# ygtxr1997/MSML

Measured on AMD Instinct MI355X. Metric: images/sec (112x112) ires50-MSML+PartialFC training step, higher is better.
Workload: dtype bf16; 1 GPU; iresnet50-MSML (OSB r18 + FM x4) + 85742-id ArcFace PartialFC, 112x112, batch 256/GPU, fwd+bwd+clip+SGD; global_batch=256, parallelism=dp1+class-parallel head, launch=eager, weight gradients + OSB on side streams

## Files before the change

include/msml_hip.h:

```cpp
#ifndef MSML_HIP_H
#define MSML_HIP_H

#include <stddef.h>
#include <stdint.h>

#ifdef __cplusplus
extern "C" {
#endif

#define MSML_ABI_VERSION 1

enum { MSML_F32 = 0, MSML_BF16 = 1, MSML_BF16X3 = 2 };

enum {
  MSML_OK = 0,
  MSML_ERR_SHAPE = -1,
  MSML_ERR_DTYPE = -2,
  MSML_ERR_LAUNCH = -3,
  MSML_ERR_UNSUPPORTED = -4,
  MSML_ERR_WORKSPACE = -5
};

enum { MSML_ACT_TANH = 0, MSML_ACT_SIGMOID = 1 };
enum { MSML_ARITH_ADD = 0, MSML_ARITH_SUB = 1, MSML_ARITH_MUL = 2, MSML_ARITH_DIV = 3 };
// ... 88 lines not shown
                          int accumulate, long M, int C, const void* next_x, const float* next_mean,
                          const float* next_invstd, double* next_acc, int dtype, void* stream);
int msml_bn_act_bwd_acc(const void* dy, const void* x, const float* scale, const float* shift,
                        const float* alpha, const float* save_mean, const float* save_invstd,
                        const void* residual_first, const void* add, void* dx, void* dres, float* dgamma,
                        float* dbeta, float* dalpha, int accumulate, long M, int C, double* acc, int dtype,
                        void* stream);
int msml_bn_act_bwd(const void* dy, const void* x, const float* scale, const float* shift,
                    const float* alpha, const float* save_mean, const float* save_invstd,
                    const void* residual_first, void* dx, void* dres, float* dgamma, float* dbeta,
                    float* dalpha, int accumulate, long M, int C, float* workspace, long ws_floats,
                    int dtype, void* stream);
int msml_bias_grad(const void* dy, long M, int Cp, int Creal, float* db, int accumulate,
                   float* workspace, long ws_floats, int dtype, void* stream);
int msml_add(const void* a, const void* b, void* out, long n, int dtype, void* stream);

int msml_dap_fwd(const void* x, float* seg, unsigned char* mask, int N, int H, int W, int Cp,
                 int dtype, void* stream);
int msml_dap_bwd(const float* dseg, void* dx, int N, int H, int W, int Cp, int dtype, void* stream);
int msml_seg_consensus_loss(const float* logit, const long* msk, int N, int H, int W, float alpha,
                            float beta, float* loss, float* dlogit, float* workspace,
                            long ws_floats, void* stream);
int msml_seg_consensus_loss_r(const float* logit, const long* msk, int N, int H, int W, float alpha, float beta,
                              int reduce_pixel_all, int reduce_pixel_kl_all, float* loss, float* dlogit,
                              float* workspace, long ws_floats, void* stream);

int msml_rownorm_fwd(const float* w, int R, int Rp, int E, void* dst, int ld, float* inv_norm,
                     int dtype, void* stream);
int msml_rownorm_bwd(const float* w, const float* inv_norm, const float* dy, int ldy, int R, int E,
                     float* dw, int accumulate, void* stream);
int msml_gather_target(const float* cosm, int ld, const long* label, int N, float* out,
                       void* stream);
int msml_margin_fwd(float* cosm, const long* label, int N, int C, int ld, int kind, float s,
                    float m, float a, float k, void* stream);
int msml_margin_bwd(const float* dlogit, int ldg, const long* label, const float* cos_t, int N,
                    int C, void* dcos, int ldo, int kind, float s, float m, float a, float k,
                    int dtype, void* stream);
int msml_pfc_rowstats(const float* cosm, int ld, int N, int C, const long* label, int kind, float s,
                      float m, float a, float k, float* rowmax, float* rowsum, void* stream);
int msml_pfc_grad(const float* cosm, int ld, int N, int C, const long* label, int kind, float s,
                  float m, float a, float k, const float* gmax, const float* gsum, float eps_ls,
                  float inv_n, void* dcos, int ldo, float* ptarget, int dtype, void* stream);
int msml_sgd_momentum(float* w, const float* grad, float* mom, long n, float lr, float mu, float wd,
                      int first_step, const float* clip_coef, void* stream);
int msml_grad_norm_clip(const float* grad, long n, float max_norm, float* out2, float* workspace,
                        long ws_floats, void* stream);
int msml_sgd_momentum_dev(float* w, const float* grad, float* mom, long n, const float* lr, float mu, float wd,
                          const float* coef, void* stream);
int msml_grad_norm_clip_scaled(const float* grad, long n, float max_norm, float scale, float* out2, float* workspace,
                               long ws_floats, void* stream);

long msml_gemm_splitk_workspace(int M, int coutp, int K);
int msml_gemm_splitk(const void* a, int M, int K, const void* wp, int kop, float* out, int coutp,
                     void* workspace, long ws_bytes, int dtype, void* stream);

int msml_pack_weights_batched(const long* table, int count, int dtype, void* stream);
int msml_pack_tiles(int A, int B, int R, int S);
int msml_pack_weights_tiled(const long* table, const int* tile_prefix, int count, int total_tiles,
                            int dtype, void* stream);

int msml_transpose(const void* src, int R, int C, int ld_s, void* dst, int ld_d, int dtype,
                   void* stream);

int msml_conv2d_fused(const void* in0, int c0p, const void* in1, int c1p, const void* wp, int kop,
                      const float* scale, const float* shift, const float* alpha,
                      const void* residual, int res_first, void* out, int coutp, int N, int H,
                      int W, int P, int Q, int R, int S, int stride, int pad_h, int pad_w,
                      int transposed, void* stream);

int msml_conv2d_x3(const void* in0, int c0p, const void* in1, int c1p, const void* wp, int kop,
                   const float* scale, const float* shift, const float* alpha, const void* residual,
                   int res_first, void* out, int coutp, int N, int H, int W, int P, int Q, int R, int S,
                   int stride, int pad_h, int pad_w, int transposed, void* stream);
int msml_conv2d_x3_border(const void* in0, int c0p, const void* wp, int kop, const float* scale,
                          const float* shift9, const float* alpha, const void* residual, int res_first,
                          void* out, int coutp, int N, int H, int W, void* stream);
int msml_x3_bn_act_fwd(const void* x, const float* scale, const float* shift, const float* alpha,
                       const void* residual, int res_first, void* y, long M, int C, void* stream);
int msml_x3_fm_fuse_fwd(const void* x, const void* yf, void* z, long M, int C, int act, int arith,
                        void* stream);
int msml_x3_add(const void* a, const void* b, void* out, long M, int C, void* stream);
int msml_x3_from_f32(const float* src, void* dst, long M, int C, void* stream);
int msml_x3_to_f32(const void* src, float* dst, long M, int C, void* stream);

int msml_pair_sqdist(const float* emb, int n_pairs, int E, double* dist, void* stream);
int msml_pair_sqdist_f64(const double* emb, int n_pairs, int E, double* dist, void* stream);
int msml_pair_hist(const double* dist, const unsigned char* same, int n_pairs, const double* thr, int nthr,
                   int nfolds, int* hist, void* stream);

int msml_occ_draw(long seed, long offset, int N, int H, int W, int mode, int lo, int hi, int flip, int* desc,
                  void* stream);
int msml_occ_apply(const unsigned char* src, const int* desc, float* img, long* msk, float* ori, int N, int H,
                   int W, int light, void* stream);

int msml_occ_draw_tex(long seed, long offset, int N, int H, int W, int mode, int lo, int hi, int flip,
                      const int* meta, int nsets, int* desc, void* stream);
int msml_occ_resize(const unsigned char* atlas, const int* meta, const int* dir, const int* rtab, const int* desc,
                    unsigned char* patch, long patch_stride, int N, int lds_bytes, void* stream);
int msml_occ_apply_tex(const unsigned char* src, const int* desc, const unsigned char* patch, long patch_stride,
                       float* img, long* msk, float* ori, int N, int H, int W, int light, void* stream);

int msml_deconv4_bwd_data(const void* dy, const void* wp0, const void* wp1, void* dx0, void* dx1, int N, int H,
                          void* stream);

int msml_conv2d_bnbwd_rows(int coutp, int N, int P, int Q);
int msml_conv2d_bnbwd(const void* in0, int c0p, const void* wp, int kop, void* out, int coutp,
                      int N, int H, int W, int P, int Q, int R, int S, int stride, int pad_h,
                      int pad_w, int transposed, const void* bn_x, const float* bn_scale,
                      const float* bn_shift, const float* bn_alpha, const float* bn_mean,
                      const float* bn_invstd, float* partial, int rows_cap, int* rows_used,
                      void* stream);
int msml_bn_act_bwd_apply(const void* dy, const void* x, const float* scale, const float* shift,
                          const float* alpha, const float* save_mean, const float* save_invstd,
                          const float* partial, int rows, const void* add, void* dx,
                          float* dgamma, float* dbeta, float* dalpha, int accumulate, long M,
                          int C, float* coef_ws, int dtype, void* stream);

int msml_bn_act_bwd_apply_s2(const void* dy, const void* x, const float* scale, const float* shift,
                             const float* alpha, const float* save_mean, const float* save_invstd,
                             const float* partial, int rows, const void* add, int H, int W, void* dx,
                             float* dgamma, float* dbeta, float* dalpha, int accumulate, long M,
                             int C, float* coef_ws, int dtype, void* stream);
int msml_bn_act_bwd_apply_next_s2(const void* dy, const void* x, const float* scale,
                                  const float* shift, const float* alpha, const float* save_mean,
                                  const float* save_invstd, const float* partial, int rows,
                                  const void* add, int H, int W, void* dx, float* dgamma, float* dbeta,
                                  float* dalpha, int accumulate, long M, int C, float* coef_ws,
                                  const void* next_x, const float* next_mean,
                                  const float* next_invstd, float* next_partial, int dtype,
                                  void* stream);

int msml_conv2d_bnin_applies(int c0p, int coutp, int N, int H, int W, int P, int Q, int R, int S,
                             int stride, int pad_h, int pad_w, int want_stats);
int msml_conv2d_bnin(const void* in0, int c0p, const float* in_scale, const float* in_shift,
                     const float* in_alpha, const void* wp, int kop, void* out, int coutp,
                     float* stats, int N, int H, int W, int P, int Q, int R, int S, int stride,
                     int pad_h, int pad_w, void* stream);
int msml_conv_wgrad_bnin_applies(int up, int vp, int A, int Breal, int N, int H, int W, int P, int Q,
                                 int R, int S, int stride, int pad_h, int pad_w);
int msml_conv_wgrad_bnin(const void* u, int up, const void* v, int vp, const float* x_scale,
                         const float* x_shift, const float* x_alpha, float* dw, int A, int Breal,
                         int Btot, int boff, int N, int H, int W, int P, int Q, int R, int S,
                         int stride, int pad_h, int pad_w, int accumulate, void* workspace,
                         long ws_bytes, void* stream);

#define MSML_KERNEL_MFM 2
const char* msml_conv2d_kernel(int c0p, int c1p, int coutp, int N, int H, int W, int P, int Q,
                               int R, int S, int stride, int pad_h, int pad_w, int transposed,
                               int in_dtype, int out_dtype, int want_stats);

int msml_stem_im2col(const float* x, void* out, int N, int C, int H, int W, int P, int Q, int R,
                     int S, int stride, int pad, int KP, int dtype, void* stream);

int msml_bn_act_bwd_apply_rows(long M, int C);
int msml_bn_act_bwd_apply_next(const void* dy, const void* x, const float* scale, const float* shift,
                               const float* alpha, const float* save_mean, const float* save_invstd,
                               const float* partial, int rows, const void* add, void* dx,
                               float* dgamma, float* dbeta, float* dalpha, int accumulate, long M,
                               int C, float* coef_ws, const void* next_x, const float* next_mean,
                               const float* next_invstd, float* next_partial, int dtype, void* stream);

int msml_conv2d_bnin_acc_applies(int c0p, int coutp, int N, int H, int W, int P, int Q, int R, int S, int stride,
                                 int pad_h, int pad_w);
int msml_conv2d_bnin_acc(const void* in0, int c0p, const double* acc_in, double count, const float* gamma,
                         const float* beta, float* running_mean, float* running_var, float momentum, float eps,
                         float* coef_out, const float* in_alpha, void* act_out, const void* wp, int kop, void* out,
                         int coutp, double* acc_out, int N, int H, int W, int P, int Q, int R, int S, int stride,
                         int pad_h, int pad_w, void* stream);

int msml_iblock_fwd_tables(int* nptr, int* nint, int* nflt);
int msml_iblock_fwd(const void* const* ptrs, const int* ints, const float* flts, void* stream);

int msml_probe_mfma(const void* seed, float* out, int wgs, int iters, void* stream);
int msml_probe_mfma_lds(const void* seed, float* out, int wgs, int iters, void* stream);


int msml_conv2d_mfm(const void* in0, int c0p, const void* wp, int kop, const float* bias, void* out, int coutp,
                    const void* residual, unsigned char* sel, int N, int H, int W, int P, int Q, int R, int S,
                    int stride, int pad_h, int pad_w, int dtype, void* stream);

int msml_mfm_bwd(const void* dy, const unsigned char* sel, void* dz, long M, int cp, int C, int czp, int dtype,
                 void* stream);

int msml_pool2_fwd(const void* x, void* y, int N, int H, int W, int cp, int dtype, void* stream);

int msml_pool2_bwd(const void* dy, const void* x, void* dx, int N, int H, int W, int cp, int dtype, void* stream);

int msml_template_pool(const float* feats, long n_rows, long ld, int E, int flip, const float* faceness,
                       const int* order, const int* media_start, const int* tmpl_media_start, const int* launch,
                       int n_templates, double* out, void* stream);
int msml_template_pair_score(const double* tn, int n_templates, int E, const int* r1, const int* r2, long n_pairs,
                             double* score, void* stream);
int msml_roc_blocks(int n);
int msml_roc_block_counts(const double* sorted, const unsigned char* label, int n, int* blk, void* stream);
int msml_roc_points(const double* sorted, const unsigned char* label, int n, const int* off, int* tps, int* fps,
                    void* stream);
int msml_roc_reduce_blocks(int n_points);
int msml_roc_reduce(const int* tps, const int* fps, int n_points, const double* target, int n_targets,
                    unsigned char* keep, unsigned long long* part, void* stream);
int msml_pair_cosdist(const float* emb, int n_pairs, int E, double* dist, void* stream);
int msml_pair_cosdist_f64(const double* emb, int n_pairs, int E, double* dist, void* stream);
int msml_rank_count(const double* sorted, int n, const double* q, int m, int strict, int* out, void* stream);

#ifdef __cplusplus
}
#endif
#endif
```

msml_amd/functional.py:

```python
import os
import torch

from . import _lib, ops
from ._lib import BF16, DTYPE_OF, F32, TORCH_DTYPE, call
from .ops import cpad


class _ToNHWC(torch.autograd.Function):

    @staticmethod
    def forward(ctx, x, dtype):
        return ops.to_nhwc(x.float(), dtype)

    @staticmethod
    def backward(ctx, g):
        return None, None


def to_nhwc(x, dtype):
    return _ToNHWC.apply(x, dtype)


def _slice_w(w, deconv, off, n):
    if deconv:
# ... 589 lines not shown
        e = weight.shape[0]
        dtype = DTYPE_OF[x.dtype]
        wp = ops.PACKS.get(weight, False, 0, e, 0, c, c, 0, dtype, owner=grad_param)
        xf = x.reshape(n, h * w * c)
        if dtype == BF16:
            y = ops.gemm_splitk(xf, wp, cpad(e))
        else:
            y, _ = ops.conv2d(x, None, wp, None, cpad(e), h, w, 1, 0, 0, False, out_dtype=F32)
            y = y.reshape(n, cpad(e))
        y = y[:, :e] + bias.detach()
        ctx.save_for_backward(x, weight, bias)
        ctx.grad_param = grad_param
        ctx.wp = wp
        return y.contiguous().reshape(n, 1, 1, e)

    @staticmethod
    def backward(ctx, dy):
        x, weight, bias = ctx.saved_tensors
        n, h, w, c = x.shape
        e = weight.shape[0]
        dtype = DTYPE_OF[x.dtype]
        dy = dy.contiguous().to(x.dtype)
        k = h * w * c
        dx = None
        if ctx.needs_input_grad[0]:
            if dtype == BF16:
                wpt = torch.empty(k, ops.kpad(e), dtype=x.dtype, device=x.device)
                call("msml_transpose", ctx.wp, e, k, k, wpt, ops.kpad(e), dtype)
                dxf, _ = ops.conv2d(dy, None, wpt, None, k, 1, 1, 1, 0, 0, False, real=(e, k))
                dx = dxf.reshape(n, h, w, c)
            else:
                wt = ops.PACKS.get(weight, True, 0, e, 0, c, e, 0, dtype, owner=ctx.grad_param)
                dx, _ = ops.conv2d(dy, None, wt, None, c, h, w, 1, 0, 0, True, p=h, q=w, real=(e, c))
        gp = ctx.grad_param
        inplace = ops.inplace(gp)
        dw = gp.grad.view(weight.shape) if inplace else torch.empty_like(weight)
        ops.conv_wgrad(dy, x, dw, e, c, c, 0, h, w, 1, 0, 0, accumulate=inplace)
        binplace = ops.inplace(bias)
        rows = ops.bn_stats_rows(n, e)
        wsb = ops.workspace(rows * 2 * e * 4, dy.device)
        db = bias.grad if binplace else torch.empty(e, dtype=torch.float32, device=dy.device)
        call("msml_bias_grad", dy, n, e, e, db, int(binplace), wsb, wsb.numel() // 4, dtype)
        if binplace:
            ops.grad_ready(bias)
            db = None
        if inplace:
            ops.grad_ready(gp)
            dw = None
        return dx, dw, db, None


def flat_fc(x, weight4d, bias, grad_param):
    return _FlatFc.apply(x, weight4d, bias, grad_param)


def _eval_bn_coef(bn_m, c):
    stamp = (bn_m.weight._version, bn_m.bias._version, bn_m.running_mean._version,
             bn_m.running_var._version, ops.WEIGHT_EPOCH, bn_m.weight.data_ptr())
    hit = getattr(bn_m, "_msml_eval_coef", None)
    if hit is None or hit[0] != stamp:
        coef = torch.empty(2, c, dtype=torch.float32, device=bn_m.weight.device)
        call("msml_bn_finalize", None, 0, c, 0.0, bn_m.weight, bn_m.bias, bn_m.running_mean,
             bn_m.running_var, 0.1, bn_m.eps, coef[0], coef[1], None, None)
        hit = (stamp, coef)
        bn_m._msml_eval_coef = hit
    return hit[1]


def conv_bn_eval(x0, x1, conv_m, bn_m, prelu, residual, c1, res_first):
    n, h, w, c0p = x0.shape
    cin, cout = conv_m.in_channels, conv_m.out_channels
    c0 = cin - c1
    r, s = conv_m.kernel_size
    stride, (ph, pw) = conv_m.stride[0], conv_m.padding
    coutp = cpad(cout)
    assert coutp == cout == bn_m.num_features
    wp = ops.PACKS.get(conv_m.weight, False, 0, cout, 0, cin, c0, c1, BF16)
    coef = _eval_bn_coef(bn_m, coutp)
    p = ops.conv_out_size(h, r, stride, ph, False)
    q = ops.conv_out_size(w, s, stride, pw, False)
    c1p = 0 if x1 is None else x1.shape[3]
    out = torch.empty(n, p, q, coutp, dtype=torch.bfloat16, device=x0.device)
    name = "conv_fused"
    if ops.PROFILE.on:
        name = ops.conv_label("N+bn", c0p, c1p, coutp, n, h, w, p, q, r, s, stride, ph, pw, 0, BF16, BF16, False)
    with ops.PROFILE.rec(name, 2.0 * n * p * q * cin * cout * r * s):
        call("msml_conv2d_fused", x0, c0p, x1, c1p, wp, wp.shape[0], coef[0], coef[1],
             prelu.weight if prelu is not None else None, residual, int(res_first), out, coutp,
             n, h, w, p, q, r, s, stride, ph, pw, 0)
    return out


class RawImage:

    def __init__(self, x, x3=False):
        self.raw = x
        self.dtype = torch.bfloat16
        self.x3 = x3
        self._nhwc = None

    def nhwc(self):
        if self._nhwc is None:
            self._nhwc = to_nhwc(self.raw, BF16)
        return self._nhwc

    def record_stream(self, stream):
        self.raw.record_stream(stream)


def _stem_pack(conv_m):
    w = conv_m.weight
    stamp = (w._version, ops.WEIGHT_EPOCH, w.data_ptr())
    hit = getattr(conv_m, "_msml_stem_pack", None)
    if hit is None or hit[0] != stamp:
        cout, cin, r, s = w.shape
        w2 = w.detach().permute(0, 2, 3, 1).reshape(cout, r * s * cin, 1, 1).contiguous()
        hit = (stamp, ops.pack_weight(w2, False, r * s * cin, 0, BF16))
        conv_m._msml_stem_pack = hit
    return hit[1]


class _StemConv(torch.autograd.Function):

    @staticmethod
    def forward(ctx, weight, conv_m, raw):
        cout, cin, r, s = weight.shape
        col = ops.stem_im2col(raw, r, s, conv_m.stride[0], conv_m.padding[0])
        wp = _stem_pack(conv_m)
        y, stats = ops.conv2d(col, None, wp, None, cpad(cout), 1, 1, 1, 0, 0, False, want_stats=True,
                              real=(r * s * cin, cout))
        ctx.set_materialize_grads(False)
        ctx.wparam = weight
        ctx.save_for_backward(col)
        ctx.mark_non_differentiable(stats)
        return y, stats

    @staticmethod
    def backward(ctx, dy, _dstats):
        if dy is None:
            return None, None, None
        (col,) = ctx.saved_tensors
        w = ctx.wparam
        cout, cin, r, s = w.shape
        k = r * s * cin
        dw2 = torch.empty(cout, k, 1, 1, dtype=torch.float32, device=dy.device)
        ops.conv_wgrad(dy.contiguous(), col, dw2, cout, k, k, 0, 1, 1, 1, 0, 0)
        dw = dw2.view(cout, r, s, cin).permute(0, 3, 1, 2)
        if ops.inplace(w):
            w.grad.view(w.shape).add_(dw)
            ops.grad_ready(w)
            return None, None, None
        return dw.contiguous(), None, None


def stem_conv_bn(raw, conv_m, bn_m, prelu):
    if raw.x3:
        return stem_conv_bn_x3(raw, conv_m, bn_m, prelu)
    if not bn_m.training and not torch.is_grad_enabled():
        cout, cin, r, s = conv_m.weight.shape
        col = ops.stem_im2col(raw.raw, r, s, conv_m.stride[0], conv_m.padding[0])
        wp = _stem_pack(conv_m)
        coef = _eval_bn_coef(bn_m, cpad(cout))
        n, p, q, kp = col.shape
        out = torch.empty(n, p, q, cpad(cout), dtype=torch.bfloat16, device=col.device)
        name = "conv_fused"
        if ops.PROFILE.on:
            name = ops.conv_label("N+bn", kp, 0, cpad(cout), n, p, q, p, q, 1, 1, 1, 0, 0, 0, BF16, BF16, False)
        with ops.PROFILE.rec(name, 2.0 * n * p * q * r * s * cin * cout):
            call("msml_conv2d_fused", col, kp, None, 0, wp, wp.shape[0], coef[0], coef[1],
                 prelu.weight if prelu is not None else None, None, 0, out, cpad(cout), n, p, q, p, q, 1, 1,
                 1, 0, 0, 0)
        return out
    y, stats = _StemConv.apply(conv_m.weight, conv_m, raw.raw)
    return bn_act(y, stats if stats.numel() else None, bn_m, prelu, emit_stats=True)


class SplitT:
    __slots__ = ("t", "c")
    dtype = "bf16x3"

    def __init__(self, t, c):
        self.t, self.c = t, c

    @property
    def shape(self):
        n, h, w, _ = self.t.shape
        return (n, h, w, self.c)

    @property
    def device(self):
        return self.t.device

    def detach(self):
        return self

    def record_stream(self, stream):
        self.t.record_stream(stream)

    def numel(self):
        n, h, w, _ = self.t.shape
        return n * h * w * self.c


def _x3_empty(n, h, w, cp, dev):
    return SplitT(torch.empty(n, h, w, 3 * cp, dtype=torch.bfloat16, device=dev), cp)


def x3_from_f32(x):
    n, h, w, cp = x.shape
    out = _x3_empty(n, h, w, cp, x.device)
    call("msml_x3_from_f32", x.contiguous(), out.t, n * h * w, cp)
    return out


def x3_to_f32(s):
    n, h, w, cp = s.shape
    out = torch.empty(n, h, w, cp, dtype=torch.float32, device=s.device)
    call("msml_x3_to_f32", s.t, out, n * h * w, cp)
    return out


def to_nchw_any(t, c):
    if isinstance(t, SplitT):
        t = x3_to_f32(t)
    return ops.to_nchw(t, c)


def _x3_expand(w, axis, segs):
    parts = []
    off = 0
    for c, cp_ in segs:
        ws = w.narrow(axis, off, c)
        if cp_ != c:
            pad = list(ws.shape)
            pad[axis] = cp_ - c
            ws = torch.cat((ws, ws.new_zeros(pad)), axis)
        wh = ws.to(torch.bfloat16).float()
        parts += [wh, wh, ws - wh]
        off += c
    return torch.cat(parts, axis).contiguous()


def _x3_pack(owner, key, w, transpose, segs):
    stamp = (w._version, ops.WEIGHT_EPOCH, w.data_ptr(), key)
    cache = owner.__dict__.setdefault("_msml_x3_pack", {})
    hit = cache.get(key)
    if hit is None or hit[0] != stamp:
        wexp = _x3_expand(w.detach().float(), 0 if transpose else 1, segs)
        c1 = 3 * segs[0][1]
        c2 = 3 * segs[1][1] if len(segs) > 1 else 0
        hit = (stamp, ops.pack_weight(wexp, transpose, c1, c2, BF16, stored=True))
        cache[key] = hit
    return hit[1]


def conv_x3(x0, x1, conv_m, scale, shift, alpha, residual, res_first, c1=0, weight=None, pack_key="fwd"):
    import torch.nn as nn
    deconv = isinstance(conv_m, nn.ConvTranspose2d)
    w = conv_m.weight if weight is None else weight
    cin, cout = conv_m.in_channels, conv_m.out_channels
    c0 = cin - c1
    r, s = conv_m.kernel_size
    stride, (ph, pw) = conv_m.stride[0], conv_m.padding
    n, h, wd, c0p = x0.shape
    segs = [(c0, c0p)] + ([(c1, x1.shape[3])] if x1 is not None else [])
    wp = _x3_pack(conv_m, pack_key, w, deconv, segs)
    coutp = cpad(cout)
    p = ops.conv_out_size(h, r, stride, ph, deconv)
    q = ops.conv_out_size(wd, s, stride, pw, deconv)
    out = _x3_empty(n, p, q, coutp, x0.device)
    pix = n * h * wd if deconv else n * p * q
    name = "conv_x3"
    if ops.PROFILE.on and os.environ.get("MSML_PROFILE_X3_SHAPES"):
        name = "conv_x3 c%d+%d->%d %dx%d k%dx%d s%d%s n%d" % (c0p, x1.shape[3] if x1 is not None else 0, coutp, h, wd, r, s,
                                                             stride, "T" if deconv else "", n)
    with ops.PROFILE.rec(name, 2.0 * pix * cin * cout * r * s):
        call("msml_conv2d_x3", x0.t, c0p, x1.t if x1 is not None else None, x1.shape[3] if x1 is not None else 0,
             wp, wp.shape[0], scale, shift, alpha, residual.t if residual is not None else None, int(res_first),
             out.t, coutp, n, h, wd, p, q, r, s, stride, ph, pw, int(deconv))
    return out


def _pad_vec(v, cp):
    if v.numel() == cp:
        return v.detach()
    out = torch.zeros(cp, dtype=torch.float32, device=v.device)
    out[:v.numel()] = v.detach()
    return out


def conv_bn_eval_x3(x0, x1, conv_m, bn_m, prelu, residual, c1, res_first):
    coutp = cpad(conv_m.out_channels)
    coef = _eval_bn_coef(bn_m, coutp)
    return conv_x3(x0, x1, conv_m, coef[0], coef[1], prelu.weight if prelu is not None else None, residual,
                   res_first, c1)


X3_FOLD_BN1 = os.environ.get("MSML_X3_NO_BN1_FOLD") is None
X3_FOLD_MAX_RATIO = 8.0


def _bn_stamp(bn_m):
    return (bn_m.weight._version, bn_m.bias._version, bn_m.running_mean._version, bn_m.running_var._version,
            bn_m.weight.data_ptr())


def bn_conv_bn_eval_x3(x, bn_in, conv_m, bn_m, prelu):
    n, h, w, cp = x.shape
    cout, cin = conv_m.out_channels, conv_m.in_channels
    if (not X3_FOLD_BN1 or conv_m.kernel_size != (3, 3) or conv_m.stride != (1, 1) or conv_m.padding != (1, 1)
            or conv_m.bias is not None or h < 2 or w < 2):
        return None
    coutp = cpad(cout)
    cw = conv_m.weight
    stamp = (_bn_stamp(bn_in), _bn_stamp(bn_m), cw._version, cw.data_ptr(), ops.WEIGHT_EPOCH, cp)
    hit = conv_m.__dict__.get("_msml_x3_fold")
    if hit is None or hit[0] != stamp:
        ratio = float((bn_in.running_mean.detach().abs() / (bn_in.running_var.detach() + bn_in.eps).sqrt()).max())
        if not ratio <= X3_FOLD_MAX_RATIO:
            conv_m.__dict__["_msml_x3_fold"] = (stamp, None, None)
            return None
        c_in = _eval_bn_coef(bn_in, cp).double()
        c_out = _eval_bn_coef(bn_m, coutp).double()
        wd = cw.detach().double()
# ... 370 lines not shown
```

Measured before the change: 8791 images/sec.

## Fuse stem conv with BN/PReLU via recompute-from-image kernels for fwd and bwd

Adds a dedicated stem kernel family that computes the 3x3x3->64 conv from the raw fp32 image with MFMA and uses it in four passes: a stats pass, a BN+PReLU apply pass, a backward-sums pass, and a backward pass that also does the weight gradient. The conv output is never stored; it is recomputed in each pass, so the im2col buffer and the conv-output tensor round trips to memory go away. The cost is running the tiny conv up to four times and adding a partial-sum reduce kernel for dW. The path is on by default and is limited to stem shapes with W <= 128.

```diff
diff --git a/include/msml_hip.h b/include/msml_hip.h
--- a/include/msml_hip.h
+++ b/include/msml_hip.h
@@ -264,6 +264,21 @@
 int msml_stem_im2col(const float* x, void* out, int N, int C, int H, int W, int P, int Q, int R,
                      int S, int stride, int pad, int KP, int dtype, void* stream);
 
+int msml_stem_part_rows(int N, int P, int Q);
+int msml_stem_stats(const float* img, const void* wp, int ktot, int N, int H, int W, int P, int Q, int stride,
+                    double* acc, void* stream);
+int msml_stem_bn_act_fwd(const float* img, const void* wp, int ktot, int N, int H, int W, int P, int Q,
+                         int stride, const double* acc, const float* gamma, const float* beta,
+                         float* running_mean, float* running_var, float momentum, float eps, float* coef,
+                         const float* alpha, void* x, double* acc_out, void* stream);
+int msml_stem_bn_bwd_sums(const float* img, const void* wp, int ktot, int N, int H, int W, int P, int Q,
+                          int stride, const void* dx, const float* coef, const float* alpha, double* acc,
+                          void* stream);
+int msml_stem_bn_bwd_wgrad(const float* img, const void* wp, int ktot, int N, int H, int W, int P, int Q,
+                           int stride, const void* dx, const float* coef, const float* alpha,
+                           const double* acc, float* dgamma, float* dbeta, float* dalpha, int accumulate,
+                           float* part, int part_rows, float* dw, int dw_accumulate, void* stream);
+
 int msml_bn_act_bwd_apply_rows(long M, int C);
 int msml_bn_act_bwd_apply_next(const void* dy, const void* x, const float* scale, const float* shift,
                                const float* alpha, const float* save_mean, const float* save_invstd,
diff --git a/msml_amd/csrc/stem.hip b/msml_amd/csrc/stem.hip
--- /dev/null
+++ b/msml_amd/csrc/stem.hip
@@ -0,0 +1,486 @@
+#include "common.h"
+
+enum { ST_STATS = 1, ST_FWD = 2, ST_BSUMS = 3, ST_BWG = 4 };
+
+struct StemArgs {
+  const float* img;
+  const unsigned short* wp;
+  int ktot;
+  int N, H, W, P, Q, stride;
+  int M;
+  int nblk;
+  double* stats;
+  BnIn bn;
+  unsigned short* x;
+  double* xacc;
+  const unsigned short* gout;
+  BnBwdFuse bnb;
+  float* dgamma;
+  float* dbeta;
+  float* dalpha;
+  int accumulate;
+  float* part;
+};
+
+#define STEM_TAB 0
+#define STEM_RED 2048
+#define STEM_SCR0 (2048 + 3072)
+#define STEM_XOUT 4096
+#define STEM_SCR (4096 + 2048)
+#define STEM_LDS (STEM_SCR0 + 4 * STEM_SCR)
+
+template <int MODE>
+__global__ void __launch_bounds__(256, 2) k_stem(const StemArgs p) {
+#if defined(__HIP_DEVICE_COMPILE__)
+  extern __shared__ __attribute__((aligned(16))) char smem[];
+  float* tab = reinterpret_cast<float*>(smem + STEM_TAB);
+  float* red = reinterpret_cast<float*>(smem + STEM_RED);
+  const int t = threadIdx.x, lane = t & 63, wave = t >> 6;
+  const int r32 = lane & 31, h = lane >> 5;
+  char* xout = smem + STEM_SCR0 + wave * STEM_SCR;
+  char* xin = xout + STEM_XOUT;
+  MSML_LDS_REGION(tab, 3 * 64 * 4);
+  MSML_LDS_REGION(red, 4 * 3 * 64 * 4);
+  MSML_LDS_REGION(xout, STEM_SCR);
+  auto key = [](int row) -> int { return (row >> 2) & 3; };
+
+  if (MODE == ST_FWD) {
+    bn_in_fill_acc(p.bn, tab, 64, t, 256, blockIdx.x == 0);
+    __syncthreads();
+  }
+  if (MODE == ST_BWG) {
+    const double* acc = reinterpret_cast<const double*>(p.bnb.partial);
+    if (t < 64) {
+      double s0 = 0.0, s1 = 0.0, s2 = 0.0;
+#pragma unroll
+      for (int r = 0; r < MSML_ACC_ROWS; r++) {
+        s0 += acc[(r * 3 + 0) * 64 + t];
+        s1 += acc[(r * 3 + 1) * 64 + t];
+        s2 += acc[(r * 3 + 2) * 64 + t];
+      }
+      tab[t] = (float)(s0 / (double)p.M);
+      tab[64 + t] = (float)(s1 / (double)p.M);
+      if (blockIdx.x == 0) {
+        if (p.dbeta) p.dbeta[t] = (p.accumulate ? p.dbeta[t] : 0.f) + (float)s0;
+        if (p.dgamma) p.dgamma[t] = (p.accumulate ? p.dgamma[t] : 0.f) + (float)s1;
+        if (p.dalpha) p.dalpha[t] = (p.accumulate ? p.dalpha[t] : 0.f) + (float)s2;
+      }
+    }
+    __syncthreads();
+  }
+
+  u32x4 wa[2][2];
+#pragma unroll
+  for (int i = 0; i < 2; i++)
+#pragma unroll
+    for (int kk = 0; kk < 2; kk++)
+      wa[i][kk] = *reinterpret_cast<const u32x4*>(p.wp + (long)(32 * i + r32) * p.ktot + (kk * 2 + h) * 8);
+
+  const int HW = p.H * p.W, PQ = p.P * p.Q;
+  const float rcpPQ = 1.0f / (float)PQ, rcpQ = 1.0f / (float)p.Q;
+
+  const int opl = lane >> 3;
+  const int cl = (lane & 7) ^ opl;
+  const bool has_alpha = MODE == ST_FWD ? p.bn.alpha != nullptr : p.bnb.alpha != nullptr;
+  float fsc[8], fsh[8], fal[8];
+  float k1[8], k2[8], bmu[8];
+  BnbCoef bk;
+  if (MODE == ST_FWD) {
+#pragma unroll
+    for (int j = 0; j < 8; j++) {
+      fsc[j] = tab[cl * 8 + j];
+      fsh[j] = tab[64 + cl * 8 + j];
+      fal[j] = tab[128 + cl * 8 + j];
+    }
+  }
+  if (MODE == ST_BSUMS || MODE == ST_BWG) bk = bnb_load_coef(p.bnb, cl * 8);
+  if (MODE == ST_BWG) {
+#pragma unroll
+    for (int j = 0; j < 8; j++) {
+      k1[j] = tab[cl * 8 + j];
+      k2[j] = tab[64 + cl * 8 + j];
+      bmu[j] = p.bnb.mean[cl * 8 + j];
+    }
+  }
+
+  f32x4 s1[MODE == ST_STATS ? 8 : 1], s2[MODE == ST_STATS ? 8 : 1];
+#pragma unroll
+  for (int g = 0; g < (MODE == ST_STATS ? 8 : 1); g++) s1[g] = s2[g] = f32x4{0.f, 0.f, 0.f, 0.f};
+  float bq[3][8];
+#pragma unroll
+  for (int q = 0; q < 3; q++)
+#pragma unroll
+    for (int j = 0; j < 8; j++) bq[q][j] = 0.f;
+  f32x16 dw[2];
+#pragma unroll
+  for (int i = 0; i < 2; i++)
+#pragma unroll
+    for (int e = 0; e < 16; e++) dw[i][e] = 0.f;
+
+  const int gw = blockIdx.x * 4 + wave, tw = gridDim.x * 4;
+  const int nunits = (p.nblk + 1) / 2;
+  for (int u = gw; u < nunits; u += tw) {
+#pragma unroll 1
+    for (int b = 0; b < 2; b++) {
+      const int pb = (u * 2 + b) * 32;
+      if (pb >= p.M) break;
+      u32x4 e2[(MODE == ST_BSUMS || MODE == ST_BWG) ? 4 : 1];
+      if (MODE == ST_BSUMS || MODE == ST_BWG) {
+#pragma unroll
+        for (int j = 0; j < 4; j++) {
+          const int m = pb + j * 8 + opl;
+          e2[j] = m < p.M ? *reinterpret_cast<const u32x4*>(p.gout + (long)m * 64 + cl * 8) : u32x4{0, 0, 0, 0};
+        }
+      }
+      const int m = pb + r32;
+      const bool valid = m < p.M;
+      const int mm = valid ? m : 0;
+      int n = (int)((float)mm * rcpPQ), rem = mm - n * PQ;
+      if (rem < 0) { n--; rem += PQ; } else if (rem >= PQ) { n++; rem -= PQ; }
+      int oy = (int)((float)rem * rcpQ), ox = rem - oy * p.Q;
+      if (ox < 0) { oy--; ox += p.Q; } else if (ox >= p.Q) { oy++; ox -= p.Q; }
+      const int iy0 = oy * p.stride - 1, ix0 = ox * p.stride - 1;
+      unsigned int colm = 0, okmask = 0;
+#pragma unroll
+      for (int s = 0; s < 3; s++) colm |= ((unsigned)(ix0 + s) < (unsigned)p.W ? 1u : 0u) << s;
+#pragma unroll
+      for (int r = 0; r < 3; r++) okmask |= ((unsigned)(iy0 + r) < (unsigned)p.H ? colm : 0u) << (3 * r);
+      if (!valid) okmask = 0;
+      const int base = n * 3 * HW + iy0 * p.W + ix0;
+      u32x4 xb[2];
+#pragma unroll
+      for (int kk = 0; kk < 2; kk++) {
+        float f[8];
+#pragma unroll
+        for (int e = 0; e < 8; e++) {
+          const int ka = kk * 16 + e, kb = kk * 16 + 8 + e;
+          const int ta = ka / 3, tb = kb / 3;
+          const int offa = (ka - ta * 3) * HW + (ta / 3) * p.W + (ta % 3);
+          const int offb = tb < 9 ? (kb - tb * 3) * HW + (tb / 3) * p.W + (tb % 3) : 0;
+          const int tap = h ? (tb < 9 ? tb : 31) : ta;
+          const bool ok = (okmask >> tap) & 1u;
+          const int idx = ok ? base + (h ? offb : offa) : 0;
+          const float v = p.img[idx];
+          f[e] = ok ? v : 0.f;
+        }
+#pragma unroll
+        for (int e = 0; e < 4; e++) xb[kk][e] = (unsigned int)f2bf(f[2 * e]) | ((unsigned int)f2bf(f[2 * e + 1]) << 16);
+      }
+      f32x16 acc[2];
+#pragma unroll
+      for (int i = 0; i < 2; i++)
+#pragma unroll
+        for (int e = 0; e < 16; e++) acc[i][e] = 0.f;
+#pragma unroll
+      for (int kk = 0; kk < 2; kk++)
+#pragma unroll
+        for (int i = 0; i < 2; i++)
+          acc[i] = __builtin_amdgcn_mfma_f32_32x32x16_bf16(__builtin_bit_cast(bf16x8, wa[i][kk]),
+                                                           __builtin_bit_cast(bf16x8, xb[kk]), acc[i], 0, 0, 0);
+      if (MODE == ST_STATS) {
+#pragma unroll
+        for (int i = 0; i < 2; i++)
+#pragma unroll
+          for (int g = 0; g < 4; g++)
+#pragma unroll
+            for (int j = 0; j < 4; j++) {
+              const float v = acc[i][g * 4 + j];
+              if (valid) {
+                s1[4 * i + g][j] += v;
+                s2[4 * i + g][j] += v * v;
+              }
+            }
+        continue;
+      }
+#pragma unroll
+      for (int i = 0; i < 2; i++) {
+        u32x2 pk[4];
+#pragma unroll
+        for (int g = 0; g < 4; g++) {
+          pk[g][0] = (unsigned int)f2bf(acc[i][g * 4 + 0]) | ((unsigned int)f2bf(acc[i][g * 4 + 1]) << 16);
+          pk[g][1] = (unsigned int)f2bf(acc[i][g * 4 + 2]) | ((unsigned int)f2bf(acc[i][g * 4 + 3]) << 16);
+        }
+        u32x4 ch[2];
+#pragma unroll
+        for (int e = 0; e < 2; e++) {
+          auto r01 = __builtin_amdgcn_permlane32_swap(pk[0][e], pk[1][e], false, false);
+          auto r23 = __builtin_amdgcn_permlane32_swap(pk[2][e], pk[3][e], false, false);
+          ch[0][e] = r01[0]; ch[0][2 + e] = r01[1];
+          ch[1][e] = r23[0]; ch[1][2 + e] = r23[1];
+        }
+#pragma unroll
+        for (int c = 0; c < 2; c++)
+          *reinterpret_cast<u32x4*>(xout + r32 * 128 + (((4 * i + 2 * c + h) ^ (r32 & 7)) << 4)) = ch[c];
+      }
+      if (MODE == ST_BWG) {
+#pragma unroll
+        for (int kk = 0; kk < 2; kk++)
+          *reinterpret_cast<u32x4*>(xin + r32 * 64 + (((kk * 2 + h) ^ key(r32)) << 4)) = xb[kk];
+      }
+      __builtin_amdgcn_wave_barrier();
+#pragma unroll
+      for (int j = 0; j < 4; j++) {
+        const int mo = pb + j * 8 + opl;
+        u32x4 v = *reinterpret_cast<const u32x4*>(xout + (j * 64 + lane) * 16);
+        const Vec8 y = load8<unsigned short>(reinterpret_cast<const unsigned short*>(&v));
+        if (MODE == ST_FWD) {
+          if (mo < p.M) {
+            Vec8 o;
+#pragma unroll
+            for (int q = 0; q < 8; q++) {
+              float z = y.v[q] * fsc[q] + fsh[q];
+              if (has_alpha) z = z > 0.f ? z : z * fal[q];
+              o.v[q] = z;
+            }
+            store8<unsigned short>(p.x + (long)mo * 64 + cl * 8, o);
+            const Vec8 vr = round8<unsigned short>(o);
+#pragma unroll
+            for (int q = 0; q < 8; q++) {
+              bq[0][q] += vr.v[q];
+              bq[1][q] += vr.v[q] * vr.v[q];
+            }
+          }
+        }
+        if (MODE == ST_BSUMS) {
+          if (mo < p.M) bnb_accum(bk, has_alpha, load8<unsigned short>(reinterpret_cast<const unsigned short*>(&e2[j])), y, bq);
+        }
+        if (MODE == ST_BWG) {
+          const Vec8 g = load8<unsigned short>(reinterpret_cast<const unsigned short*>(&e2[j]));
+          Vec8 o;
+#pragma unroll
+          for (int q = 0; q < 8; q++) {
+            float gg = g.v[q];
+            if (has_alpha) {
+              const float z = y.v[q] * bk.sc[q] + bk.sh[q];
+              if (z <= 0.f) gg *= bk.al[q];
+            }
+            const float xh = (y.v[q] - bmu[q]) * bk.is[q];
+            o.v[q] = mo < p.M ? bk.sc[q] * (gg - k1[q] - xh * k2[q]) : 0.f;
+          }
+          u32x4 w;
+          store8<unsigned short>(reinterpret_cast<unsigned short*>(&w), o);
+          *reinterpret_cast<u32x4*>(xout + (j * 64 + lane) * 16) = w;
+        }
+      }
+      if (MODE == ST_BWG) {
+        __builtin_amdgcn_wave_barrier();
+#pragma unroll
+        for (int st = 0; st < 2; st++) {
+          u32x4 bf, af[2];
+#pragma unroll
+          for (int e = 0; e < 8; e += 2) {
+            unsigned int lo[3], hi[3];
+#pragma unroll
+            for (int d = 0; d < 2; d++) {
+              const int px = st * 16 + h * 8 + e + d;
+              const unsigned int vb = *reinterpret_cast<const unsigned short*>(xin + px * 64 + (((r32 >> 3) ^ key(px)) << 4) + (r32 & 7) * 2);
+              unsigned int va[2];
+#pragma unroll
+              for (int i = 0; i < 2; i++) {
+                const int c = 32 * i + r32;
+                va[i] = *reinterpret_cast<const unsigned short*>(xout + px * 128 + (((c >> 3) ^ (px & 7)) << 4) + (c & 7) * 2);
+              }
+              if (d == 0) { lo[0] = vb; lo[1] = va[0]; lo[2] = va[1]; } else { hi[0] = vb; hi[1] = va[0]; hi[2] = va[1]; }
+            }
+            bf[e >> 1] = lo[0] | (hi[0] << 16);
+            af[0][e >> 1] = lo[1] | (hi[1] << 16);
+            af[1][e >> 1] = lo[2] | (hi[2] << 16);
+          }
+#pragma unroll
+          for (int i = 0; i < 2; i++)
+            dw[i] = __builtin_amdgcn_mfma_f32_32x32x16_bf16(__builtin_bit_cast(bf16x8, af[i]), __builtin_bit_cast(bf16x8, bf),
+                                                            dw[i], 0, 0, 0);
+        }
+      }
+      __builtin_amdgcn_wave_barrier();
+    }
+  }
+
+  if (MODE == ST_STATS) {
+#pragma unroll
+    for (int g = 0; g < 8; g++)
+#pragma unroll
+      for (int j = 0; j < 4; j++) {
+        const float a = wave_half_sum(s1[g][j]), b2 = wave_half_sum(s2[g][j]);
+        if (r32 == 0) {
+          red[(wave * 2 + 0) * 64 + 8 * g + 4 * h + j] = a;
+          red[(wave * 2 + 1) * 64 + 8 * g + 4 * h + j] = b2;
+        }
+      }
+    __syncthreads();
+    for (int e = t; e < 2 * 64; e += 256) {
+      const int q = e / 64, c = e % 64;
+      float sum = 0.f;
+#pragma unroll
+      for (int w = 0; w < 4; w++) sum += red[(w * 2 + q) * 64 + c];
+      stats_emit(reinterpret_cast<float*>(p.stats), 1, blockIdx.x, q, 64, c, sum);
+    }
+  }
+  if ((MODE == ST_FWD && p.xacc) || MODE == ST_BSUMS) {
+    constexpr int NQ = MODE == ST_FWD ? 2 : 3;
+#pragma unroll
+    for (int q = 0; q < NQ; q++)
+#pragma unroll
+      for (int j = 0; j < 8; j++) {
+        float a = bq[q][j];
+        a += __shfl_xor(a, 9, 64);
+        a += __shfl_xor(a, 18, 64);
+        a += __shfl_xor(a, 36, 64);
+        if (lane < 8) red[(wave * NQ + q) * 64 + 8 * cl + j] = a;
+      }
+    __syncthreads();
+    for (int e = t; e < NQ * 64; e += 256) {
+      const int q = e / 64, c = e % 64;
+      float sum = 0.f;
+#pragma unroll
+      for (int w = 0; w < 4; w++) sum += red[(w * NQ + q) * 64 + c];
+      if (MODE == ST_FWD) stats_emit(reinterpret_cast<float*>(p.xacc), 1, blockIdx.x, q, 64, c, sum);
+      else bnb_emit(p.bnb.partial, 1, blockIdx.x, q, 64, c, sum);
+    }
+  }
+  if (MODE == ST_BWG) {
+    float* tile = reinterpret_cast<float*>(smem + STEM_SCR0);
+    __syncthreads();
+    for (int w = 0; w < 4; w++) {
+      if (wave == w) {
+#pragma unroll
+        for (int i = 0; i < 2; i++)
+#pragma unroll
+          for (int g = 0; g < 4; g++)
+#pragma unroll
+            for (int j = 0; j < 4; j++) {
+              const int idx = (32 * i + 8 * g + 4 * h + j) * 32 + r32;
+              tile[idx] = (w ? tile[idx] : 0.f) + dw[i][g * 4 + j];
+            }
+      }
+      __syncthreads();
+    }
+    float* dst = p.part + (long)blockIdx.x * 2048;
+    for (int e = t; e < 2048; e += 256) dst[e] = tile[e];
+  }
+#endif
+}
+
+__global__ void __launch_bounds__(1024) k_stem_wgrad_reduce(const float* __restrict__ part, int rows, float* __restrict__ dw,
+                                                            int accumulate) {
+  __shared__ float red[32][33];
+  const int co = blockIdx.x, k = threadIdx.x & 31, sl = threadIdx.x >> 5;
+  float s = 0.f;
+  for (int r = sl; r < rows; r += 32) s += part[(long)r * 2048 + co * 32 + k];
+  red[sl][k] = s;
+  __syncthreads();
+  if (sl == 0 && k < 27) {
+    float sum = 0.f;
+#pragma unroll
+    for (int i = 0; i < 32; i++) sum += red[i][k];
+    const int tap = k / 3, c = k - tap * 3;
+    float* d = dw + co * 27 + c * 9 + tap;
+    *d = (accumulate ? *d : 0.f) + sum;
+  }
+}
+
+static int stem_cus() {
+  static int cus = 0;
+  if (!cus) {
+    int dev = 0, n = 256;
+    if (hipGetDevice(&dev) == hipSuccess) (void)hipDeviceGetAttribute(&n, hipDeviceAttributeMultiprocessorCount, dev);
+    cus = n > 0 ? n : 256;
+  }
+  return cus;
+}
+
+static int stem_grid(long M) {
+  const long nblk = (M + 31) / 32, nunits = (nblk + 1) / 2;
+  long grid = (long)stem_cus() * 4;
+  const long need = (nunits + 3) / 4;
+  if (grid > need) grid = need;
+  return (int)(grid < 1 ? 1 : grid);
+}
+
+static int stem_fill(StemArgs& a, const char* who, const float* img, const void* wp, int ktot, int N, int H, int W, int P,
+                     int Q, int stride) {
+  MSML_CHECK(img && wp && N > 0 && H > 0 && W > 0 && ktot >= 32, MSML_ERR_SHAPE, "%s: bad arguments", who);
+  MSML_CHECK((stride == 1 || stride == 2) && P == (H + 2 - 3) / stride + 1 && Q == (W + 2 - 3) / stride + 1 && W <= 128,
+             MSML_ERR_UNSUPPORTED, "%s: 3x3 / pad 1 / stride 1 or 2 / W <= 128 only (H=%d W=%d P=%d Q=%d stride=%d)", who,
+             H, W, P, Q, stride);
+  const long M = (long)N * P * Q;
+  MSML_CHECK(M < (1L << 24) && (long)N * 3 * H * W < (1L << 29), MSML_ERR_UNSUPPORTED, "%s: N*P*Q = %ld must be < 2^24", who, M);
+  a = StemArgs{};
+  a.img = img; a.wp = (const unsigned short*)wp; a.ktot = ktot;
+  a.N = N; a.H = H; a.W = W; a.P = P; a.Q = Q; a.stride = stride;
+  a.M = (int)M; a.nblk = (int)((M + 31) / 32);
+  return MSML_OK;
+}
+
+extern "C" int msml_stem_part_rows(int N, int P, int Q) { return stem_grid((long)N * P * Q); }
+
+extern "C" int msml_stem_stats(const float* img, const void* wp, int ktot, int N, int H, int W, int P, int Q, int stride,
+                               double* acc, void* stream) {
+  StemArgs a;
+  const int rc = stem_fill(a, "stem_stats", img, wp, ktot, N, H, W, P, Q, stride);
+  if (rc != MSML_OK) return rc;
+  MSML_CHECK(acc, MSML_ERR_SHAPE, "stem_stats: null accumulator");
+  a.stats = acc;
+  k_stem<ST_STATS><<<stem_grid(a.M), 256, STEM_LDS, (hipStream_t)stream>>>(a);
+  MSML_LAUNCH_OK("stem_stats");
+  return MSML_OK;
+}
+
+extern "C" int msml_stem_bn_act_fwd(const float* img, const void* wp, int ktot, int N, int H, int W, int P, int Q,
+                                    int stride, const double* acc, const float* gamma, const float* beta,
+                                    float* running_mean, float* running_var, float momentum, float eps, float* coef,
+                                    const float* alpha, void* x, double* acc_out, void* stream) {
+  StemArgs a;
+  const int rc = stem_fill(a, "stem_bn_act_fwd", img, wp, ktot, N, H, W, P, Q, stride);
+  if (rc != MSML_OK) return rc;
+  MSML_CHECK(acc && coef && x, MSML_ERR_SHAPE, "stem_bn_act_fwd: null argument");
+  a.bn.acc = acc; a.bn.count = (double)a.M; a.bn.gamma = gamma; a.bn.beta = beta;
+  a.bn.rmean = running_mean; a.bn.rvar = running_var; a.bn.momentum = momentum; a.bn.eps = eps;
+  a.bn.coef_out = coef; a.bn.alpha = alpha;
+  a.x = (unsigned short*)x; a.xacc = acc_out;
+  k_stem<ST_FWD><<<stem_grid(a.M), 256, STEM_LDS, (hipStream_t)stream>>>(a);
+  MSML_LAUNCH_OK("stem_bn_act_fwd");
+  return MSML_OK;
+}
+
+static void stem_bnb(StemArgs& a, const void* dx, const float* coef, const float* alpha, double* acc) {
+  a.gout = (const unsigned short*)dx;
+  a.bnb.x = nullptr;
+  a.bnb.scale = coef; a.bnb.shift = coef + 64; a.bnb.mean = coef + 128; a.bnb.invstd = coef + 192;
+  a.bnb.alpha = alpha;
+  a.bnb.partial = reinterpret_cast<float*>(acc);
+  a.bnb.acc = 1;
+}
+
+extern "C" int msml_stem_bn_bwd_sums(const float* img, const void* wp, int ktot, int N, int H, int W, int P, int Q,
+                                     int stride, const void* dx, const float* coef, const float* alpha, double* acc,
+                                     void* stream) {
+  StemArgs a;
+  const int rc = stem_fill(a, "stem_bn_bwd_sums", img, wp, ktot, N, H, W, P, Q, stride);
+  if (rc != MSML_OK) return rc;
+  MSML_CHECK(dx && coef && acc, MSML_ERR_SHAPE, "stem_bn_bwd_sums: null argument");
+  stem_bnb(a, dx, coef, alpha, acc);
+  k_stem<ST_BSUMS><<<stem_grid(a.M), 256, STEM_LDS, (hipStream_t)stream>>>(a);
+  MSML_LAUNCH_OK("stem_bn_bwd_sums");
+  return MSML_OK;
+}
+
+extern "C" int msml_stem_bn_bwd_wgrad(const float* img, const void* wp, int ktot, int N, int H, int W, int P, int Q,
+                                      int stride, const void* dx, const float* coef, const float* alpha,
+                                      const double* acc, float* dgamma, float* dbeta, float* dalpha, int accumulate,
+                                      float* part, int part_rows, float* dw, int dw_accumulate, void* stream) {
+  StemArgs a;
+  const int rc = stem_fill(a, "stem_bn_bwd_wgrad", img, wp, ktot, N, H, W, P, Q, stride);
+  if (rc != MSML_OK) return rc;
+  const int grid = stem_grid(a.M);
+  MSML_CHECK(dx && coef && acc && part && dw, MSML_ERR_SHAPE, "stem_bn_bwd_wgrad: null argument");
+  MSML_CHECK(part_rows >= grid, MSML_ERR_SHAPE, "stem_bn_bwd_wgrad: %d partial rows, %d needed", part_rows, grid);
+  stem_bnb(a, dx, coef, alpha, const_cast<double*>(acc));
+  a.dgamma = dgamma; a.dbeta = dbeta; a.dalpha = dalpha; a.accumulate = accumulate;
+  a.part = part;
+  k_stem<ST_BWG><<<grid, 256, STEM_LDS, (hipStream_t)stream>>>(a);
+  MSML_LAUNCH_OK("stem_bn_bwd_wgrad");
+  k_stem_wgrad_reduce<<<64, 1024, 0, (hipStream_t)stream>>>(part, grid, dw, dw_accumulate);
+  MSML_LAUNCH_OK("stem_wgrad_reduce");
+  return MSML_OK;
+}
diff --git a/msml_amd/functional.py b/msml_amd/functional.py
--- a/msml_amd/functional.py
+++ b/msml_amd/functional.py
@@ -765,6 +765,97 @@
             return None, None, None
         return dw.contiguous(), None, None
 
+STEM_FUSED = os.environ.get("MSML_STEM_FUSED", "1") != "0"
+_STEM_ROWS = {}
+
+
+def _stem_fused_applies(raw, conv_m, bn_m):
+    if not (STEM_FUSED and bn_m.training and raw.dtype == torch.bfloat16 and ops.acc_applies(64, BF16)):
+        return False
+    x = raw.raw
+    if x.dim() != 4 or x.dtype != torch.float32 or tuple(conv_m.weight.shape) != (64, 3, 3, 3) or conv_m.bias is not None:
+        return False
+    n, c, h, w = x.shape
+    stride = conv_m.stride[0]
+    if (c != 3 or tuple(conv_m.padding) != (1, 1) or tuple(conv_m.stride) != (stride, stride) or stride not in (1, 2)
+            or tuple(conv_m.dilation) != (1, 1) or conv_m.groups != 1 or w > 128):
+        return False
+    p, q = ops.conv_out_size(h, 3, stride, 1, False), ops.conv_out_size(w, 3, stride, 1, False)
+    return (bn_m.num_features == 64 and bn_m.weight is not None and bn_m.bias is not None
+            and bn_m.running_mean is not None and n * p * q < (1 << 24) and x.numel() < (1 << 29))
+
+
+class _StemFused(torch.autograd.Function):
+
+    @staticmethod
+    def forward(ctx, weight, gamma, beta, alpha, conv_m, bn_m, raw, emit):
+        n, _, h, w = raw.shape
+        stride = conv_m.stride[0]
+        p, q = ops.conv_out_size(h, 3, stride, 1, False), ops.conv_out_size(w, 3, stride, 1, False)
+        dims = (n, h, w, p, q, stride)
+        dev = raw.device
+        img = raw.contiguous()
+        wp = _stem_pack(conv_m)
+        ktot = wp.shape[1]
+        nx = n * p * q * 64 * 2
+        acc = ops.stats_acc(64, dev)
+        with ops.PROFILE.rec("bn_act_fwd", 0.0, img.numel() * 4):
+            call("msml_stem_stats", img, wp, ktot, *dims, acc)
+        coef = torch.empty(4, 64, dtype=torch.float32, device=dev)
+        x = torch.empty(n, p, q, 64, dtype=torch.bfloat16, device=dev)
+        xacc = ops.stats_acc(64, dev) if emit else None
+        with ops.PROFILE.rec("bn_act_fwd", 0.0, img.numel() * 4 + nx):
+            call("msml_stem_bn_act_fwd", img, wp, ktot, *dims, acc, gamma, beta, bn_m.running_mean, bn_m.running_var,
+                 0.1 if bn_m.momentum is None else bn_m.momentum, bn_m.eps, coef, alpha, x, xacc)
+        ctx.dims, ctx.wp = dims, wp
+        ctx.params = (weight, gamma, beta, alpha)
+        ctx.set_materialize_grads(False)
+        ctx.save_for_backward(img, coef, alpha)
+        if emit:
+            ctx.mark_non_differentiable(xacc)
+            return x, xacc
+        return x
+
+    @staticmethod
+    def backward(ctx, gx, *_dacc):
+        if gx is None:
+            return (None,) * 8
+        img, coef, alpha = ctx.saved_tensors
+        weight, gamma, beta, alpha_p = ctx.params
+        n, h, w, p, q, stride = ctx.dims
+        wp, dev = ctx.wp, img.device
+        gx = gx.contiguous()
+        nx = gx.numel() * 2
+        bacc = ops.stats_acc(64, dev, 3)
+        with ops.PROFILE.rec("bn_act_bwd", 0.0, img.numel() * 4 + nx):
+            call("msml_stem_bn_bwd_sums", img, wp, wp.shape[1], *ctx.dims, gx, coef, alpha, bacc)
+        rows = _STEM_ROWS.get((n, p, q))
+        if rows is None:
+            rows = _STEM_ROWS[(n, p, q)] = _lib.value("msml_stem_part_rows", n, p, q)
+        part = ops.workspace(rows * 8192, dev, "stem")
+        want = (ctx.needs_input_grad[1], ctx.needs_input_grad[2], alpha is not None and ctx.needs_input_grad[3])
+        inplace = all((not wt) or ops.inplace(prm) for wt, prm in zip(want, (gamma, beta, alpha_p)))
+        pg = None
+        if inplace:
+            tg = [prm.grad if wt else None for wt, prm in zip(want, (gamma, beta, alpha_p))]
+        else:
+            pg = torch.empty(3, 64, dtype=torch.float32, device=dev)
+            tg = [pg[0], pg[1], pg[2] if alpha is not None else None]
+        w_inplace = ctx.needs_input_grad[0] and ops.inplace(weight)
+        dw = weight.grad if w_inplace else torch.empty(64, 3, 3, 3, dtype=torch.float32, device=dev)
+        with ops.PROFILE.rec("bn_act_bwd", 0.0, img.numel() * 4 + nx):
+            call("msml_stem_bn_bwd_wgrad", img, wp, wp.shape[1], *ctx.dims, gx, coef, alpha, bacc, tg[0], tg[1], tg[2],
+                 int(inplace), part, rows, dw, int(w_inplace))
+        if inplace:
+            ops.grad_ready(*[prm for wt, prm in zip(want, (gamma, beta, alpha_p)) if wt])
+        if w_inplace:
+            ops.grad_ready(weight)
+        return (dw if ctx.needs_input_grad[0] and not w_inplace else None,
+                pg[0] if want[0] and not inplace else None,
+                pg[1] if want[1] and not inplace else None,
+                pg[2] if want[2] and not inplace else None,
+                None, None, None, None)
+
 
 def stem_conv_bn(raw, conv_m, bn_m, prelu):
     if raw.x3:
@@ -783,6 +874,16 @@
             call("msml_conv2d_fused", col, kp, None, 0, wp, wp.shape[0], coef[0], coef[1],
                  prelu.weight if prelu is not None else None, None, 0, out, cpad(cout), n, p, q, p, q, 1, 1,
                  1, 0, 0, 0)
+        return out
+    if _stem_fused_applies(raw, conv_m, bn_m):
+        ops.bn_counter(bn_m)
+        emit = bool(ops.EMIT_STEM_STATS)
+        out = _StemFused.apply(conv_m.weight, bn_m.weight, bn_m.bias, prelu.weight if prelu is not None else None,
+                               conv_m, bn_m, raw.raw, emit)
+        if emit:
+            x, xacc = out
+            x._msml_stats = xacc
+            return x
         return out
     y, stats = _StemConv.apply(conv_m.weight, conv_m, raw.raw)
     return bn_act(y, stats if stats.numel() else None, bn_m, prelu, emit_stats=True)
```

After: 8918 images/sec (median of 4 runs). 1.01x the previous value.
